# rqhuang88/DV-Matcher

Hardware: AMD Instinct MI355X
Metric: point-cloud pairs/sec (N=2048, d=128) (higher is better)
Workload: dtype f32; 1 GPU; BASELINE configs[1]: synthetic random pairs N=M=2048 d=128, correspondence+deform forward, both directions; deformer_weights=reference ckpt/dvmatcher_scape_r (fixture), fps_start=0, parallelism=pairs sharded over 1 GPU(s), no collective

## Files before the change

dv-matcher_amd/csrc/dvm_grid.hip:

```cpp
#include <stdlib.h>

#include <type_traits>

#include "dvm_common.h"
#include "dvm_mlp_f16.h"

namespace dvm {

constexpr int GRID_T = 256;

template <class IndexT>
struct GridViewT {
    const float4 *pts;
    const IndexT *ids;
    const IndexT *start;
    float ox, oy, oz, h, scale2;
    int G;
};
typedef GridViewT<int32_t> GridView;
typedef GridViewT<uint16_t> GridViewLds;


static int grid_dim_for(int P) {
    int g = 2;
    while (g < 16 && (double)(g + 1) * (g + 1) * (g + 1) * 1.2 <= (double)P * 1.15) ++g;
    return g < 4 ? 4 : g;
}

struct GridBuildSets {
    const float *xyz[4];
    int Nsrc[4];
    GridBuf gb[4];
};
template <bool SETS>
__device__ __forceinline__ void grid_build_body(const float *__restrict__ xyz, int Nsrc, const int32_t *__restrict__ sel, const GridBuf &gb);
__global__ __launch_bounds__(GRID_T) void grid_build_sets_kernel(const GridBuildSets sets) {
    const int q = blockIdx.y;
    grid_build_body<true>(sets.xyz[q], sets.Nsrc[q], nullptr, sets.gb[q]);
}
__global__ __launch_bounds__(GRID_T) void grid_build_kernel(const float *__restrict__ xyz, int Nsrc,
                                                            const int32_t *__restrict__ sel, GridBuf gb) {
    grid_build_body<false>(xyz, Nsrc, sel, gb);
}
template <bool SETS>
__device__ __forceinline__ void grid_build_body(const float *__restrict__ xyz, int Nsrc, const int32_t *__restrict__ sel, const GridBuf &gb) {
    extern __shared__ int lds[];
    __shared__ float red[6][GRID_T / 64];
    __shared__ float par[8];
    __shared__ int wsum[GRID_T / 64];
    const int b = blockIdx.x, tid = threadIdx.x, lane = tid & 63, wave = tid >> 6;
    const int P = gb.P, G = gb.G, G3 = G * G * G;
    const float *p = xyz + (size_t)b * Nsrc * 3;
    const int32_t *sl = sel ? sel + (size_t)b * P : nullptr;
    constexpr int GC = 8;
    const bool cached = P <= GC * GRID_T;
    float px[GC], py[GC], pz[GC];
    if (cached) {
        int vs[GC];
#pragma unroll
        for (int q = 0; q < GC; ++q) {
            const int j = tid + q * GRID_T, jc = j < P ? j : P - 1;
            vs[q] = sl ? sl[jc] : jc;
        }
#pragma unroll
        for (int q = 0; q < GC; ++q) px[q] = p[3 * vs[q]], py[q] = p[3 * vs[q] + 1], pz[q] = p[3 * vs[q] + 2];
    }
    auto each_point = [&](auto &&f) __attribute__((always_inline)) {
        if (cached) {
#pragma unroll
            for (int q = 0; q < GC; ++q) {
                const int j = tid + q * GRID_T;
                if (j < P) f(j, px[q], py[q], pz[q]);
            }
        } else {
            for (int j = tid; j < P; j += GRID_T) {
                const int v = sl ? sl[j] : j;
                f(j, p[3 * v], p[3 * v + 1], p[3 * v + 2]);
            }
        }
    };
    float mn[3] = {INFINITY, INFINITY, INFINITY}, mx[3] = {-INFINITY, -INFINITY, -INFINITY};
    each_point([&](int, float x, float y, float z) {
        mn[0] = fminf(mn[0], x), mn[1] = fminf(mn[1], y), mn[2] = fminf(mn[2], z);
        mx[0] = fmaxf(mx[0], x), mx[1] = fmaxf(mx[1], y), mx[2] = fmaxf(mx[2], z);
    });
    for (int a = 0; a < 3; ++a) {
        for (int o = 32; o > 0; o >>= 1) {
            mn[a] = fminf(mn[a], __shfl_xor(mn[a], o, 64));
            mx[a] = fmaxf(mx[a], __shfl_xor(mx[a], o, 64));
        }
        if (lane == 0) {
            red[a][wave] = mn[a];
            red[3 + a][wave] = mx[a];
        }
    }
    __syncthreads();
    if (tid == 0) {
        float lo[3], hi[3];
        for (int a = 0; a < 3; ++a) {
            lo[a] = fminf(fminf(red[a][0], red[a][1]), fminf(red[a][2], red[a][3]));
            hi[a] = fmaxf(fmaxf(red[3 + a][0], red[3 + a][1]), fmaxf(red[3 + a][2], red[3 + a][3]));
        }
        float ext = fmaxf(fmaxf(hi[0] - lo[0], hi[1] - lo[1]), hi[2] - lo[2]);
        float h = ext > 0.f ? (ext / (float)G) * 1.000001f : 1.f;
        float m = 0.f;
        for (int a = 0; a < 3; ++a) m = fmaxf(m, fmaxf(fabsf(lo[a]), fabsf(hi[a])));
        par[0] = lo[0], par[1] = lo[1], par[2] = lo[2], par[3] = h, par[4] = 3.f * m * m + 1e-30f;
        for (int q = 0; q < 5; ++q) gb.params[(size_t)b * 8 + q] = par[q];
    }
    for (int c = tid; c <= G3; c += GRID_T) lds[c] = 0;
    __syncthreads();
    const float ox = par[0], oy = par[1], oz = par[2], inv = 1.0f / par[3];
    auto cell_of = [&](float x, float y, float z) {
        int cx = (int)((x - ox) * inv), cy = (int)((y - oy) * inv), cz = (int)((z - oz) * inv);
        cx = cx < 0 ? 0 : (cx > G - 1 ? G - 1 : cx);
        cy = cy < 0 ? 0 : (cy > G - 1 ? G - 1 : cy);
        cz = cz < 0 ? 0 : (cz > G - 1 ? G - 1 : cz);
        return (cz * G + cy) * G + cx;
    };
    each_point([&](int, float x, float y, float z) { atomicAdd(&lds[cell_of(x, y, z)], 1); });
    __syncthreads();
    const int chunk = (G3 + GRID_T - 1) / GRID_T;
    int local = 0;
    for (int c = tid * chunk; c < (tid + 1) * chunk && c < G3; ++c) local += lds[c];
    int inc = local;
    for (int o = 1; o < 64; o <<= 1) {
        int t = __shfl_up(inc, o, 64);
        if (lane >= o) inc += t;
    }
    if (lane == 63) wsum[wave] = inc;
    __syncthreads();
    int base = inc - local;
    for (int w2 = 0; w2 < wave; ++w2) base += wsum[w2];
    __syncthreads();
    int *cursor = lds + G3 + 1;
    int run = base;
    for (int c = tid * chunk; c < (tid + 1) * chunk && c < G3; ++c) {
        int cnt = lds[c];
        lds[c] = run;
        cursor[c] = run;
        run += cnt;
    }
    if (tid == 0) lds[G3] = P;
    __syncthreads();
    int32_t *st = gb.start + (size_t)b * (G3 + 1);
    for (int c = tid; c <= G3; c += GRID_T) st[c] = lds[c];
    float4 *op = gb.pts + (size_t)b * P;
    int32_t *oi = gb.ids + (size_t)b * P;
    each_point([&](int j, float x, float y, float z) {
        const int pos = atomicAdd(&cursor[cell_of(x, y, z)], 1);
        op[pos] = make_float4(x, y, z, sumsq3(x, y, z));
        oi[pos] = j;
    });
}

__device__ __forceinline__ GridView grid_view(const GridBuf &gb, int b) {
    GridView g;
    const int G3 = gb.G * gb.G * gb.G;
    g.pts = gb.pts + (size_t)b * gb.P;
    g.ids = gb.ids + (size_t)b * gb.P;
    g.start = gb.start + (size_t)b * (G3 + 1);
    const float *pr = gb.params + (size_t)b * 8;
    g.ox = pr[0], g.oy = pr[1], g.oz = pr[2], g.h = pr[3], g.scale2 = pr[4];
    g.G = gb.G;
    return g;
}

struct MetricMMQueryRow {
    typedef float key_t;
    float qx, qy, qz, nq;
    __device__ __forceinline__ void set(float x, float y, float z) { qx = x, qy = y, qz = z, nq = sumsq3(x, y, z); }
    __device__ __forceinline__ float operator()(const float4 &c) const {
        return sqrt_rn(d2_mm3(qx, qy, qz, nq, c.x, c.y, c.z, c.w));
    }
    __device__ __forceinline__ static float to_d2(float k) { return k * k; }
};
struct MetricMMCandRow {
    typedef float key_t;
    float qx, qy, qz, nq;
    __device__ __forceinline__ void set(float x, float y, float z) { qx = x, qy = y, qz = z, nq = sumsq3(x, y, z); }
    __device__ __forceinline__ float operator()(const float4 &c) const {
        return sqrt_rn(d2_mm3(c.x, c.y, c.z, c.w, qx, qy, qz, nq));
    }
    __device__ __forceinline__ static float to_d2(float k) { return k * k; }
};
struct MetricF64 {
    typedef double key_t;
    float qx, qy, qz;
    __device__ __forceinline__ void set(float x, float y, float z) { qx = x, qy = y, qz = z; }
    __device__ __forceinline__ double operator()(const float4 &c) const {
        double dx = (double)qx - (double)c.x, dy = (double)qy - (double)c.y, dz = (double)qz - (double)c.z;
        double s = 0.0;
        s = s + dx * dx;
        s = s + dy * dy;
        s = s + dz * dz;
        return s;
    }
    __device__ __forceinline__ static float to_d2(double k) { return (float)k; }
};
struct MetricF64Rounded {
    typedef float key_t;
    MetricF64 m;
    __device__ __forceinline__ void set(float x, float y, float z) { m.set(x, y, z); }
    __device__ __forceinline__ float operator()(const float4 &c) const { return (float)m(c); }
    __device__ __forceinline__ static float to_d2(float k) { return k; }
};
struct MetricDiff {
    typedef float key_t;
    float qx, qy, qz;
    __device__ __forceinline__ void set(float x, float y, float z) { qx = x, qy = y, qz = z; }
    __device__ __forceinline__ float operator()(const float4 &c) const { return d2_diff3(qx, qy, qz, c.x, c.y, c.z); }
    __device__ __forceinline__ static float to_d2(float k) { return k; }
};

template <class View, class Metric, class List>
__device__ __forceinline__ void grid_row(const View &g, const Metric &met, List &kb, int s0, int s1) {
    for (int s = s0; s < s1; ++s) kb.insert_lex(met(g.pts[s]), (int)g.ids[s]);
}

struct ChamferMin {
    float key;
    __device__ __forceinline__ float worst() const { return key; }
};
template <class Metric>
__device__ __forceinline__ void grid_row(const GridView &g, const Metric &met, ChamferMin &kb, int s0, int s1) {
    for (; s0 < s1; s0 += 4) {
        float4 pc[4];
#pragma unroll
        for (int u = 0; u < 4; ++u) pc[u] = g.pts[s0 + u < s1 ? s0 + u : s1 - 1];
#pragma unroll
        for (int u = 0; u < 4; ++u) kb.key = fminf(kb.key, s0 + u < s1 ? met(pc[u]) : INFINITY);
    }
}
struct ChamferMinPos {
    float key;
    int pos;
    __device__ __forceinline__ float worst() const { return key; }
};
template <class Metric>
__device__ __forceinline__ void grid_row(const GridView &g, const Metric &met, ChamferMinPos &kb, int s0, int s1) {
    for (int s = s0; s < s1; ++s) {
        const float v = met(g.pts[s]);
        if (v < kb.key) {
            kb.key = v, kb.pos = s;
        } else if (v == kb.key && (kb.pos < 0 || g.ids[s] < g.ids[kb.pos])) {
            kb.pos = s;
        }
    }
}

template <int K, class Metric, class List, class View>
__device__ __forceinline__ bool grid_search(const View &g, float qx, float qy, float qz, Metric &met, List &kb,
                                            int R0 = 1 , int Rmax = 1 << 30) {
    const int G = g.G;
    const float inv = 1.0f / g.h;
    int cx = (int)((qx - g.ox) * inv), cy = (int)((qy - g.oy) * inv), cz = (int)((qz - g.oz) * inv);
    cx = cx < 0 ? 0 : (cx > G - 1 ? G - 1 : cx);
    cy = cy < 0 ? 0 : (cy > G - 1 ? G - 1 : cy);
    cz = cz < 0 ? 0 : (cz > G - 1 ? G - 1 : cz);
    const float q2 = sumsq3(qx, qy, qz);
    const float margin = 64.f * 1.1920929e-7f * (g.scale2 + q2) + 1e-30f;
    int Rprev = R0 > 1 ? R0 - 1 : -1;
    for (int R = R0; R <= G && R <= Rmax; ++R) {
        const int x0 = cx - R < 0 ? 0 : cx - R, x1 = cx + R > G - 1 ? G - 1 : cx + R;
        const int y0 = cy - R < 0 ? 0 : cy - R, y1 = cy + R > G - 1 ? G - 1 : cy + R;
        const int z0 = cz - R < 0 ? 0 : cz - R, z1 = cz + R > G - 1 ? G - 1 : cz + R;
        for (int z = z0; z <= z1; ++z) {
            const float zlo = g.oz + (float)z * g.h;
            const float dz = fmaxf(0.f, fmaxf(zlo - qz, qz - (zlo + g.h)));
            for (int y = y0; y <= y1; ++y) {
                const float ylo = g.oy + (float)y * g.h;
                const float dy = fmaxf(0.f, fmaxf(ylo - qy, qy - (ylo + g.h)));
                if (Metric::to_d2(kb.worst()) < (dy * dy + dz * dz) * 0.9999f - margin) continue;
                const int rowbase = (z * G + y) * G;
                const bool inner_zy = (abs(z - cz) <= Rprev) && (abs(y - cy) <= Rprev);
                int sa0, sa1, sb0 = 0, sb1 = 0;
                if (inner_zy) {
                    const int ix0 = cx - Rprev < 0 ? 0 : cx - Rprev;
                    const int ix1 = cx + Rprev > G - 1 ? G - 1 : cx + Rprev;
                    sa0 = g.start[rowbase + x0];
                    sa1 = g.start[rowbase + ix0];
                    sb0 = g.start[rowbase + ix1 + 1];
                    sb1 = g.start[rowbase + x1 + 1];
                } else {
                    sa0 = g.start[rowbase + x0];
                    sa1 = g.start[rowbase + x1 + 1];
                }
                grid_row(g, met, kb, sa0, sa1);
                grid_row(g, met, kb, sb0, sb1);
            }
        }
        const float ext = (float)G * g.h;
        const float ex = fmaxf(0.f, fmaxf(g.ox - qx, qx - (g.ox + ext)));
        const float ey = fmaxf(0.f, fmaxf(g.oy - qy, qy - (g.oy + ext)));
        const float ez = fmaxf(0.f, fmaxf(g.oz - qz, qz - (g.oz + ext)));
        const float exx = ex * ex, eyy = ey * ey, ezz = ez * ez;
        float bound2 = INFINITY;
        auto face_x = [&](float f) { f = fmaxf(f, 0.f); bound2 = fminf(bound2, f * f + eyy + ezz); };
        auto face_y = [&](float f) { f = fmaxf(f, 0.f); bound2 = fminf(bound2, f * f + exx + ezz); };
        auto face_z = [&](float f) { f = fmaxf(f, 0.f); bound2 = fminf(bound2, f * f + exx + eyy); };
        if (cx - R >= 1) face_x(qx - (g.ox + (float)(cx - R) * g.h));
        if (cx + R < G - 1) face_x((g.ox + (float)(cx + R + 1) * g.h) - qx);
        if (cy - R >= 1) face_y(qy - (g.oy + (float)(cy - R) * g.h));
        if (cy + R < G - 1) face_y((g.oy + (float)(cy + R + 1) * g.h) - qy);
        if (cz - R >= 1) face_z(qz - (g.oz + (float)(cz - R) * g.h));
        if (cz + R < G - 1) face_z((g.oz + (float)(cz + R + 1) * g.h) - qz);
        if (bound2 == INFINITY) return true;
        const float kth = Metric::to_d2(kb.worst());
        if (kth < bound2 * 0.9999f - margin) return true;
        Rprev = R;
    }
    return Rmax >= G;
}

static __host__ __device__ __forceinline__ size_t grid_lds_bytes(int P, int G) {
    return ((size_t)P * (sizeof(float4) + sizeof(uint16_t)) + ((size_t)G * G * G + 1) * sizeof(uint16_t) + 15) / 16 * 16;
}
static size_t grid_lds_bytes(const GridBuf &gb) { return gb.P < 65536 ? grid_lds_bytes(gb.P, gb.G) : ~(size_t)0; }
__device__ __forceinline__ GridViewLds grid_stage_lds(const GridView &g, int P, char *lds, int threads) {
    const int G3 = g.G * g.G * g.G;
    float4 *lp = (float4 *)lds;
    uint16_t *li = (uint16_t *)(lds + (size_t)P * sizeof(float4));
    uint16_t *ls = li + P;
    for (int i = threadIdx.x; i < P; i += threads) lp[i] = g.pts[i], li[i] = (uint16_t)g.ids[i];
    for (int i = threadIdx.x; i <= G3; i += threads) ls[i] = (uint16_t)g.start[i];
    GridViewLds v;
    v.pts = lp, v.ids = li, v.start = ls;
    v.ox = g.ox, v.oy = g.oy, v.oz = g.oz, v.h = g.h, v.scale2 = g.scale2, v.G = g.G;
    return v;
}

template <int K, int THREADS = 128, bool LDS_GRID = false>
__global__ __launch_bounds__(THREADS) void grid_knn_self_kernel(GridBuf gb, int k, int32_t *__restrict__ idx) {
    extern __shared__ __attribute__((aligned(16))) char kn_lds[];
    const int b = blockIdx.y;
    const int t = blockIdx.x * blockDim.x + threadIdx.x;
    const int P = gb.P;
    const GridView gg = grid_view(gb, b);
    typename std::conditional<LDS_GRID, GridViewLds, GridView>::type g;
    if constexpr (LDS_GRID) {
        g = grid_stage_lds(gg, P, kn_lds, THREADS);
        __syncthreads();
    } else {
        g = gg;
    }
    if (t >= P) return;
    const float4 qp = g.pts[t];
    MetricMMQueryRow met;
    met.set(qp.x, qp.y, qp.z);
    KBestPacked<K> kb;
    kb.init(INFINITY);
    grid_search<K, MetricMMQueryRow>(g, qp.x, qp.y, qp.z, met, kb);
    int32_t *o = idx + ((size_t)b * P + g.ids[t]) * k;
    for (int q = 0; q < K; ++q)
        if (q < k) o[q] = (unsigned)kb.idx_at(q) < (unsigned)P ? kb.idx_at(q) : 0;
}

template <int THREADS = 128, bool LDS_GRID = false>
__global__ __launch_bounds__(THREADS) void grid_ring_kernel(GridBuf gb, int32_t *__restrict__ ring) {
    extern __shared__ __attribute__((aligned(16))) char rg_lds[];
    const int b = blockIdx.y;
    const int t = blockIdx.x * blockDim.x + threadIdx.x;
    const int P = gb.P;
    const GridView gg = grid_view(gb, b);
    typename std::conditional<LDS_GRID, GridViewLds, GridView>::type g;
    if constexpr (LDS_GRID) {
        g = grid_stage_lds(gg, P, rg_lds, THREADS);
        __syncthreads();
    } else {
        g = gg;
    }
    if (t >= P) return;
    const float4 qp = g.pts[t];
    const int a = g.ids[t];
    int32_t *o = ring + ((size_t)b * P + a) * 9;
    MetricF64Rounded mr;
    mr.set(qp.x, qp.y, qp.z);
    KBestPacked<10, 8> ks;
    ks.init(INFINITY);
    grid_search<9, MetricF64Rounded>(g, qp.x, qp.y, qp.z, mr, ks);
    bool ambiguous = false;
#pragma unroll
    for (int q = 0; q < 9; ++q) ambiguous = ambiguous || (ks.key_at(q) == ks.key_at(q + 1) && ks.key_at(q) < INFINITY);
    if (!ambiguous) {
        for (int q = 0; q < 9; ++q) o[q] = (unsigned)ks.idx_at(q) < (unsigned)P ? ks.idx_at(q) : a;
        return;
    }
    MetricF64 met;
    met.set(qp.x, qp.y, qp.z);
    KBest<9, double> kb;
    kb.init((double)INFINITY);
    grid_search<9, MetricF64>(g, qp.x, qp.y, qp.z, met, kb);
    for (int q = 0; q < 9; ++q) o[q] = (unsigned)kb.idx[q] < (unsigned)P ? kb.idx[q] : a;
}

template <int THREADS = 128, int LDS_GRID = 0>
__global__ __launch_bounds__(THREADS) void grid_infl_kernel(const float *__restrict__ xyz, int N, GridBuf gnodes, GridBuf gverts,
                                                            int32_t *__restrict__ infl, float *__restrict__ dists,
                                                            double *__restrict__ nnd) {
    extern __shared__ __attribute__((aligned(16))) char in_lds[];
    const int b = blockIdx.y;
    const int t = blockIdx.x * blockDim.x + threadIdx.x;
    const GridView gv0 = grid_view(gverts, b), gn0 = grid_view(gnodes, b);
    typename std::conditional<(LDS_GRID & 2) != 0, GridViewLds, GridView>::type gv;
    typename std::conditional<(LDS_GRID & 1) != 0, GridViewLds, GridView>::type gn;
    size_t used = 0;
    if constexpr ((LDS_GRID & 2) != 0) {
        gv = grid_stage_lds(gv0, gverts.P, in_lds, THREADS);
        used = grid_lds_bytes(gverts.P, gverts.G);
    } else {
        gv = gv0;
    }
    if constexpr ((LDS_GRID & 1) != 0) {
        gn = grid_stage_lds(gn0, gnodes.P, in_lds + used, THREADS);
    } else {
        gn = gn0;
    }
    if (LDS_GRID) __syncthreads();
    if (t >= N) return;
    const float4 qp = gv.pts[t];
    const int i = gv.ids[t];
    {
        MetricMMCandRow met;
        met.set(qp.x, qp.y, qp.z);
        KBestPacked<3> kb;
        kb.init(INFINITY);
        grid_search<3, MetricMMCandRow>(gn, qp.x, qp.y, qp.z, met, kb);
        const size_t row = (size_t)b * N + i;
        for (int q = 0; q < 3; ++q) {
            infl[row * 3 + q] = (unsigned)kb.idx_at(q) < (unsigned)gnodes.P ? kb.idx_at(q) : 0;
            dists[row * 3 + q] = kb.key_at(q);
        }
    }
    {
        MetricF64 met;
        met.set(qp.x, qp.y, qp.z);
        KBest<2, double> kb;
        kb.init((double)INFINITY);
        grid_search<2, MetricF64>(gv, qp.x, qp.y, qp.z, met, kb);
        nnd[(size_t)b * N + i] = sqrt(kb.key[1]);
    }
    (void)xyz;
}

struct ChGridGroup {
    GridBuf gq;
    GridBuf gb;
    float *dout;
    int32_t *iout;
};
struct ChGridArgs {
    ChGridGroup g[8];
    int scan_min;
    unsigned long long *stats;
};
typedef float f32x16_g __attribute__((ext_vector_type(16)));
typedef _Float16 f16x8_g __attribute__((ext_vector_type(8)));
typedef unsigned u32x4_g __attribute__((ext_vector_type(4)));

template <bool WANT_IDX>
__device__ __forceinline__ void chamfer_exact_scan(const GridView &g, const MetricDiff &met, int s_begin, int s_end, float &best, int &bs) {
    for (int s0 = s_begin; s0 < s_end; s0 += 4) {
        float4 pc[4];
#pragma unroll
        for (int u = 0; u < 4; ++u) pc[u] = g.pts[s0 + u < s_end ? s0 + u : s_end - 1];
#pragma unroll
        for (int u = 0; u < 4; ++u) {
            const int sidx = s0 + u;
            const float d = sidx < s_end ? met(pc[u]) : INFINITY;
            if (!WANT_IDX) {
                best = fminf(best, d);
            } else if (d < best) {
                best = d, bs = sidx;
            } else if (d == best && d < INFINITY && g.ids[sidx] < g.ids[bs]) {
                bs = sidx;
            }
        }
    }
}

__device__ __forceinline__ float fmin2i(float a, float b) {
    float r;
    asm("v_min_f32 %0, %1, %2" : "=v"(r) : "v"(a), "v"(b));
    return r;
}
__device__ __forceinline__ float acc_min16(const f32x16_g &acc, float inf) {
    const float last = __builtin_canonicalizef(acc[15]);
    float r0, r1, r2;
    asm("v_min3_f32 %0, %3, %4, %5\n\t"
        "v_min3_f32 %1, %6, %7, %8\n\t"
        "v_min3_f32 %2, %9, %10, %11\n\t"
        "v_min3_f32 %0, %0, %1, %2\n\t"
        "v_min3_f32 %1, %12, %13, %14\n\t"
        "v_min3_f32 %2, %15, %16, %17\n\t"
        "v_min3_f32 %1, %1, %2, %18\n\t"
        "v_min3_f32 %0, %0, %1, %19"
        : "=&v"(r0), "=&v"(r1), "=&v"(r2)
        : "v"(acc[0]), "v"(acc[1]), "v"(acc[2]), "v"(acc[3]), "v"(acc[4]), "v"(acc[5]), "v"(acc[6]), "v"(acc[7]), "v"(acc[8]),
          "v"(acc[9]), "v"(acc[10]), "v"(acc[11]), "v"(acc[12]), "v"(acc[13]), "v"(acc[14]), "v"(last), "v"(inf));
    return r0;
}
__device__ __forceinline__ float fmed3i(float a, float b, float c) {
    float r;
    asm("v_med3_f32 %0, %1, %2, %3" : "=v"(r) : "v"(a), "v"(b), "v"(c));
    return r;
}

template <bool WANT_IDX>
__device__ __forceinline__ void chamfer_scan_wave(const ChGridGroup &G, const GridView &g, int b, int Na, bool done, const float4 qp, int i,
                                                  const MetricDiff &met, float margin, unsigned long long *stats, int grp) {
    const int P = G.gb.P;
    const int lane = threadIdx.x & 63, j32 = lane & 31, hh = lane >> 5;
    if (stats) {
        if (lane == 0) atomicAdd(stats + grp * 8 + 5, 1ull);
        if (!done) atomicAdd(stats + grp * 8 + 6, 1ull);
    }
    float tb[2] = {INFINITY, INFINITY}, ts[2] = {INFINITY, INFINITY}, th[2] = {INFINITY, INFINITY};
    int tt[2] = {0, 0}, tu[2] = {0, 0};
    const float finf = INFINITY;
    auto keep = [&](int tl, float m, int s0) {
        const bool lt1 = m < tb[tl], lt2 = m < ts[tl];
        int tun = lt2 ? s0 : tu[tl];
        asm volatile("" : "+v"(tun));
        tu[tl] = lt1 ? tt[tl] : tun;
        tt[tl] = lt1 ? s0 : tt[tl];
        th[tl] = fmed3i(ts[tl], th[tl], m);
        ts[tl] = fmed3i(tb[tl], ts[tl], m);
        tb[tl] = fmin2i(tb[tl], m);
    };
    constexpr int TB = 2;
    auto fetch = [&](float4 (&buf)[TB], int s00) {
#pragma unroll
        for (int u = 0; u < TB; ++u) {
            const int pi = s00 + j32, last = P - 1 - 32 * u;
            buf[u] = g.pts[(pi < last ? pi : last) + 32 * u];
        }
    };
    auto sweep = [&](auto &&unit) {
        float4 pa[TB], pb[TB];
        fetch(pa, 0);
        for (int s00 = 0; s00 < P; s00 += 64 * TB) {
            fetch(pb, s00 + 32 * TB);
#pragma unroll
            for (int u = 0; u < TB; ++u) {
                if (s00 + 32 * u >= P) break;
                unit(pa[u], s00 + 32 * u);
            }
            fetch(pa, s00 + 64 * TB);
#pragma unroll
            for (int u = 0; u < TB; ++u) {
                if (s00 + 32 * (TB + u) >= P) break;
                unit(pb[u], s00 + 32 * (TB + u));
            }
        }
    };
    float q2m = sumsq3(qp.x, qp.y, qp.z);
#pragma unroll
    for (int o = 32; o > 0; o >>= 1) q2m = fmaxf(q2m, __shfl_xor(q2m, o, 64));
    const int r2bits = __builtin_amdgcn_readfirstlane(__float_as_int(fmaxf(g.scale2, q2m)));
    const bool f16 = r2bits < 0x7f800000;
    const int ks = (25 - ((r2bits >> 23) - 127)) >> 1;
    const float sc2 = f16 ? __int_as_float((2 * ks + 127) << 23) : 1.f;
    if (f16) {
        const float sq = __int_as_float((ks + 127) << 23), sx = -2.f * sq, sn = __int_as_float((2 * ks - 12 + 127) << 23);
        f16x8_g bq[2];
#pragma unroll
        for (int tl = 0; tl < 2; ++tl) {
            const int src = j32 + 32 * tl;
            const float x = __shfl(qp.x, src, 64), y = __shfl(qp.y, src, 64), z = __shfl(qp.z, src, 64);
            unsigned h01, m01, h23, m23;
            split2x2(sq * x, sq * y, h01, m01);
            split2x2(sq * z, 4096.f, h23, m23);
            bq[tl] = __builtin_bit_cast(f16x8_g, u32x4_g{hh ? 0u : h01, hh ? 0u : h23, hh ? m01 : h01, hh ? m23 : h23});
        }
        sweep([&](const float4 &pc, int s0) {
            unsigned h01, m01, h23, m23;
            split2x2(sx * pc.x, sx * pc.y, h01, m01);
            split2x2(sx * pc.z, sn * pc.w, h23, m23);
            const f16x8_g a = __builtin_bit_cast(f16x8_g, u32x4_g{hh ? 0u : h01, hh ? 0u : h23, hh ? h01 : m01, hh ? h23 : m23});
            const f32x16_g zero = {0.f, 0.f, 0.f, 0.f, 0.f, 0.f, 0.f, 0.f, 0.f, 0.f, 0.f, 0.f, 0.f, 0.f, 0.f, 0.f};
            const f32x16_g acc0 = __builtin_amdgcn_mfma_f32_32x32x16_f16(a, bq[0], zero, 0, 0, 0);
            const f32x16_g acc1 = __builtin_amdgcn_mfma_f32_32x32x16_f16(a, bq[1], zero, 0, 0, 0);
            keep(0, acc_min16(acc0, finf), s0);
            keep(1, acc_min16(acc1, finf), s0);
        });
    } else {
        float bq[2][2];
#pragma unroll
        for (int tl = 0; tl < 2; ++tl) {
            const int src = j32 + 32 * tl;
            const float x = __shfl(qp.x, src, 64), y = __shfl(qp.y, src, 64), z = __shfl(qp.z, src, 64);
            bq[tl][0] = hh ? -2.f * y : -2.f * x;
            bq[tl][1] = hh ? 1.f : -2.f * z;
        }
        sweep([&](const float4 &pc, int s0) {
            const float a0 = hh ? pc.y : pc.x, a1 = hh ? pc.w : pc.z;
#pragma unroll
            for (int tl = 0; tl < 2; ++tl) {
                f32x16_g acc = {0.f, 0.f, 0.f, 0.f, 0.f, 0.f, 0.f, 0.f, 0.f, 0.f, 0.f, 0.f, 0.f, 0.f, 0.f, 0.f};
                acc = __builtin_amdgcn_mfma_f32_32x32x2f32(a0, bq[tl][0], acc, 0, 0, 0);
                acc = __builtin_amdgcn_mfma_f32_32x32x2f32(a1, bq[tl][1], acc, 0, 0, 0);
                keep(tl, acc_min16(acc, finf), s0);
            }
        });
    }
    const float b1 = hh ? tb[1] : tb[0], s1 = hh ? ts[1] : ts[0], h1 = hh ? th[1] : th[0];
    const int t1 = hh ? tt[1] : tt[0], u1 = hh ? tu[1] : tu[0];
    const float b2 = __shfl_xor(hh ? tb[0] : tb[1], 32, 64), s2 = __shfl_xor(hh ? ts[0] : ts[1], 32, 64), h2 = __shfl_xor(hh ? th[0] : th[1], 32, 64);
    const int t2 = __shfl_xor(hh ? tt[0] : tt[1], 32, 64), u2 = __shfl_xor(hh ? tu[0] : tu[1], 32, 64);
    const float sbest = fminf(b1, b2);
    const int stile = b2 < b1 ? t2 : t1;
    const float c1 = t1 != stile ? b1 : INFINITY, c2 = u1 != stile ? s1 : INFINITY, c3 = t2 != stile ? b2 : INFINITY, c4 = u2 != stile ? s2 : INFINITY;
    const float ssec = fminf(fminf(c1, c2), fminf(c3, c4));
    const int stile2 = ssec == c1 ? t1 : (ssec == c2 ? u1 : (ssec == c3 ? t2 : u2));
    const float o1 = t1 != stile2 ? c1 : INFINITY, o2 = u1 != stile2 ? c2 : INFINITY, o3 = t2 != stile2 ? c3 : INFINITY, o4 = u2 != stile2 ? c4 : INFINITY;
    const float sother = fminf(fminf(h1, h2), fminf(fminf(o1, o2), fminf(o3, o4)));
    float best = INFINITY;
    int bs = 0;
    bool cert = false;
    if (!done) {
        chamfer_exact_scan<WANT_IDX>(g, met, stile, stile + 32 < P ? stile + 32 : P, best, bs);
        if (ssec < INFINITY) chamfer_exact_scan<WANT_IDX>(g, met, stile2, stile2 + 32 < P ? stile2 + 32 : P, best, bs);
        cert = sother - sbest > 2.f * (f16 ? margin * sc2 + 4.f : margin);
    }
    if (__ballot(!done && !cert) != 0) {
        if (!done && !cert) {
            if (stats) atomicAdd(stats + grp * 8 + 7, 1ull);
            best = INFINITY, bs = 0;
            chamfer_exact_scan<WANT_IDX>(g, met, 0, P, best, bs);
        }
    }
    if (!done) {
        G.dout[(size_t)b * Na + i] = best;
        if (WANT_IDX && G.iout) G.iout[(size_t)b * Na + i] = g.ids[bs];
    }
}

template <int THREADS, bool LDS_TARGET, bool WANT_IDX>
__global__ __launch_bounds__(THREADS) void grid_chamfer_kernel(const ChGridArgs args) {
    extern __shared__ __attribute__((aligned(16))) char ch_lds[];
    const ChGridGroup &G = args.g[blockIdx.z];
    const int b = blockIdx.y;
    const int t = blockIdx.x * blockDim.x + threadIdx.x;
    const int Na = G.gq.P;
    const bool inrange = t < Na;
    GridView g = grid_view(G.gb, b);
    if (LDS_TARGET) {
        const int P = G.gb.P, G3 = G.gb.G * G.gb.G * G.gb.G;
        float4 *lp = (float4 *)ch_lds;
        int32_t *ls = (int32_t *)(ch_lds + (size_t)P * sizeof(float4));
        for (int i = threadIdx.x; i < P; i += THREADS) lp[i] = g.pts[i];
        for (int i = threadIdx.x; i <= G3; i += THREADS) ls[i] = g.start[i];
        __syncthreads();
        g.pts = lp;
        g.start = ls;
    }
    GridView q = grid_view(G.gq, b);
    const int tq = inrange ? t : Na - 1;
    const float4 qp = q.pts[tq];
    const int i = q.ids[tq];
    MetricDiff met;
    met.set(qp.x, qp.y, qp.z);
    const float q2 = sumsq3(qp.x, qp.y, qp.z);
    const float margin = 64.f * 1.1920929e-7f * (g.scale2 + q2) + 1e-30f;
    bool done = !inrange;
    float fbest = INFINITY;
    int fpos = -1;
    {
        const int Gd = g.G;
        const float inv = 1.0f / g.h;
        int cx = (int)((qp.x - g.ox) * inv), cy = (int)((qp.y - g.oy) * inv), cz = (int)((qp.z - g.oz) * inv);
        cx = cx < 0 ? 0 : (cx > Gd - 1 ? Gd - 1 : cx);
        cy = cy < 0 ? 0 : (cy > Gd - 1 ? Gd - 1 : cy);
        cz = cz < 0 ? 0 : (cz > Gd - 1 ? Gd - 1 : cz);
        const int x0 = cx - 1 < 0 ? 0 : cx - 1, x1 = cx + 1 > Gd - 1 ? Gd - 1 : cx + 1;
        int rs[9], re[9];
#pragma unroll
        for (int r = 0; r < 9; ++r) {
            const int z = cz + r / 3 - 1, y = cy + r % 3 - 1;
            const bool in = z >= 0 && z < Gd && y >= 0 && y < Gd;
            const int rowbase = ((in ? z : cz) * Gd + (in ? y : cy)) * Gd;
            rs[r] = g.start[rowbase + x0];
            const int rend = g.start[rowbase + x1 + 1];
            re[r] = in ? rend : rs[r];
        }
        float best = INFINITY;
        int bs = -1;
        bool tie = false;
        const float dlo[2] = {fmaxf(0.f, qp.y - (g.oy + (float)cy * g.h)), fmaxf(0.f, qp.z - (g.oz + (float)cz * g.h))};
        const float dhi[2] = {fmaxf(0.f, (g.oy + (float)(cy + 1) * g.h) - qp.y), fmaxf(0.f, (g.oz + (float)(cz + 1) * g.h) - qp.z)};
        constexpr int order[9] = {4, 1, 3, 5, 7, 0, 2, 6, 8};
        float rowb[9];
#pragma unroll
        for (int r = 0; r < 9; ++r) {
            const float dyr = r % 3 == 1 ? 0.f : (r % 3 == 0 ? dlo[0] : dhi[0]), dzr = r / 3 == 1 ? 0.f : (r / 3 == 0 ? dlo[1] : dhi[1]);
            rowb[r] = (dyr * dyr + dzr * dzr) * 0.9999f - margin;
        }
#pragma unroll
        for (int ri = 0; ri < 9; ++ri) {
            const int r = order[ri];
            if (best < rowb[r]) continue;
            const int rend = re[r];
            for (int s0 = rs[r]; s0 < rend; s0 += 4) {
                float4 pc[4];
#pragma unroll
                for (int u = 0; u < 4; ++u) pc[u] = g.pts[s0 + u < rend ? s0 + u : rend - 1];
#pragma unroll
                for (int u = 0; u < 4; ++u) {
                    const int s = s0 + u;
                    float dm = met(pc[u]);
                    asm volatile("" : "+v"(dm));
                    const bool inb = s < rend;
                    const float d = inb ? dm : INFINITY;
                    if (WANT_IDX) {
                        const bool lt = d < best, eq = d == best && inb && d < INFINITY;
                        tie = lt ? false : (tie || eq);
                        bs = lt ? s : bs;
                        best = lt ? d : best;
                    } else {
                        best = fminf(best, d);
                    }
                }
            }
        }
        if (WANT_IDX && tie && bs >= 0) {
            int bid = g.ids[bs];
#pragma unroll 1
            for (int r = 0; r < 9; ++r) {
                if (best < rowb[r]) continue;
                for (int s = rs[r]; s < re[r]; ++s) {
                    if (met(g.pts[s]) == best) {
                        const int id = g.ids[s];
                        if (id < bid) bid = id, bs = s;
                    }
                }
            }
        }
        const float ext = (float)Gd * g.h;
        const float ex = fmaxf(0.f, fmaxf(g.ox - qp.x, qp.x - (g.ox + ext)));
        const float ey = fmaxf(0.f, fmaxf(g.oy - qp.y, qp.y - (g.oy + ext)));
        const float ez = fmaxf(0.f, fmaxf(g.oz - qp.z, qp.z - (g.oz + ext)));
        const float exx = ex * ex, eyy = ey * ey, ezz = ez * ez;
        float bound2 = INFINITY;
        auto face = [&](float f, float o2) { f = fmaxf(f, 0.f); bound2 = fminf(bound2, f * f + o2); };
        if (cx - 1 >= 1) face(qp.x - (g.ox + (float)(cx - 1) * g.h), eyy + ezz);
        if (cx + 1 < Gd - 1) face((g.ox + (float)(cx + 2) * g.h) - qp.x, eyy + ezz);
        if (cy - 1 >= 1) face(qp.y - (g.oy + (float)(cy - 1) * g.h), exx + ezz);
        if (cy + 1 < Gd - 1) face((g.oy + (float)(cy + 2) * g.h) - qp.y, exx + ezz);
        if (cz - 1 >= 1) face(qp.z - (g.oz + (float)(cz - 1) * g.h), exx + eyy);
        if (cz + 1 < Gd - 1) face((g.oz + (float)(cz + 2) * g.h) - qp.z, exx + eyy);
        if (args.stats && inrange) {
            int ncand = 0;
#pragma unroll
            for (int r = 0; r < 9; ++r) ncand += re[r] - rs[r];
            atomicAdd(args.stats + blockIdx.z * 8 + 0, 1ull);
            atomicAdd(args.stats + blockIdx.z * 8 + 1, (unsigned long long)ncand);
        }
        const bool found = WANT_IDX ? bs >= 0 : best < INFINITY;
        if (found) fbest = best, fpos = bs;
        if (!done && found && (bound2 == INFINITY || best < bound2 * 0.9999f - margin)) {
            G.dout[(size_t)b * Na + i] = best;
            if (WANT_IDX && G.iout) G.iout[(size_t)b * Na + i] = g.ids[bs];
            done = true;
            if (args.stats) atomicAdd(args.stats + blockIdx.z * 8 + 2, 1ull);
        }
    }
    const int nfall = __popcll(__ballot(!done));
    if (nfall == 0) return;
    bool scan = nfall >= args.scan_min;
    if (!scan) {
        if (!done) {
            if (args.stats) atomicAdd(args.stats + blockIdx.z * 8 + 3, 1ull);
            typename std::conditional<WANT_IDX, ChamferMinPos, ChamferMin>::type kb;
            kb.key = fbest;
            if constexpr (WANT_IDX) kb.pos = fpos;
            if (grid_search<1, MetricDiff>(g, qp.x, qp.y, qp.z, met, kb, 2, 3)) {
                if (args.stats) atomicAdd(args.stats + blockIdx.z * 8 + 4, 1ull);
                G.dout[(size_t)b * Na + i] = kb.key;
                if constexpr (WANT_IDX)
                    if (G.iout) G.iout[(size_t)b * Na + i] = kb.pos >= 0 ? g.ids[kb.pos] : 0;
                done = true;
            }
        }
        scan = __ballot(!done) != 0;
        if (!scan) return;
    }
    chamfer_scan_wave<WANT_IDX>(G, g, b, Na, done, qp, i, met, margin, args.stats, blockIdx.z);
}

GridBuf grid_carve(Arena &ar, int B, int P) {
    GridBuf gb;
    gb.P = P;
    gb.G = grid_dim_for(P);
    const int G3 = gb.G * gb.G * gb.G;
    gb.pts = ar.take<float4>((size_t)B * P);
    gb.ids = ar.take<int32_t>((size_t)B * P);
    gb.start = ar.take<int32_t>((size_t)B * (G3 + 1));
    gb.params = ar.take<float>((size_t)B * 8);
    return gb;
}
size_t grid_bytes(int B, int P) {
    Arena ar(nullptr, 0);
    grid_carve(ar, B, P);
    return ar.off;
}

void launch_grid_build_sets(const float *const *xyz, const int *Nsrc, const GridBuf *gb, int nsets, int B, hipStream_t s) {
    GridBuildSets sets;
    size_t lds = 0;
    for (int q = 0; q < 4; ++q) {
        const int r = q < nsets ? q : 0;
        sets.xyz[q] = xyz[r], sets.Nsrc[q] = Nsrc[r], sets.gb[q] = gb[r];
        const int G3 = gb[r].G * gb[r].G * gb[r].G;
        const size_t nb = (size_t)(2 * G3 + 1) * sizeof(int);
        lds = nb > lds ? nb : lds;
    }
    hipLaunchKernelGGL(grid_build_sets_kernel, dim3(B, nsets), dim3(GRID_T), lds, s, sets);
}
void launch_grid_build(const float *xyz, int B, int Nsrc, const int32_t *sel, const GridBuf &gb, hipStream_t s) {
    const int G3 = gb.G * gb.G * gb.G;
    size_t lds = (size_t)(2 * G3 + 1) * sizeof(int);
    hipLaunchKernelGGL(grid_build_kernel, dim3(B), dim3(GRID_T), lds, s, xyz, Nsrc, sel, gb);
}

template <int K>
static void launch_knn_self_k(const GridBuf &gb, int B, int k, int32_t *idx, hipStream_t s) {
    const size_t lds = grid_lds_bytes(gb);
    if (lds <= 64 * 1024) {
        ensure_dyn_lds((const void *)grid_knn_self_kernel<K, 512, true>, (int)lds);
        hipLaunchKernelGGL((grid_knn_self_kernel<K, 512, true>), dim3((gb.P + 511) / 512, B), dim3(512), lds, s, gb, k, idx);
    } else {
        hipLaunchKernelGGL((grid_knn_self_kernel<K, 128, false>), dim3((gb.P + 127) / 128, B), dim3(128), 0, s, gb, k, idx);
    }
}

void launch_grid_knn_self(const GridBuf &gb, int B, int k, int32_t *idx, hipStream_t s) {
    prof_begin(s, DVM_PROF_KNN_XYZ);
    if (k <= 3)
        launch_knn_self_k<3>(gb, B, k, idx, s);
    else if (k <= 10)
        launch_knn_self_k<10>(gb, B, k, idx, s);
    else
        launch_knn_self_k<16>(gb, B, k, idx, s);
    prof_end(s, DVM_PROF_KNN_XYZ);
}

void launch_grid_ring(const GridBuf &gnodes, int B, int32_t *ring, hipStream_t s) {
    const size_t lds = grid_lds_bytes(gnodes);
    if (lds <= 64 * 1024) {
        ensure_dyn_lds((const void *)grid_ring_kernel<512, true>, (int)lds);
        hipLaunchKernelGGL((grid_ring_kernel<512, true>), dim3((gnodes.P + 511) / 512, B), dim3(512), lds, s, gnodes, ring);
    } else {
        hipLaunchKernelGGL((grid_ring_kernel<128, false>), dim3((gnodes.P + 127) / 128, B), dim3(128), 0, s, gnodes, ring);
    }
}

void launch_grid_infl(const float *xyz, int B, int N, const GridBuf &gnodes, const GridBuf &gverts, int32_t *infl, float *dists,
                      double *nnd, hipStream_t s) {
    const size_t lds = grid_lds_bytes(gnodes);
    if (lds <= 64 * 1024) {
        ensure_dyn_lds((const void *)grid_infl_kernel<512, 1>, (int)lds);
        hipLaunchKernelGGL((grid_infl_kernel<512, 1>), dim3((N + 511) / 512, B), dim3(512), lds, s, xyz, N, gnodes, gverts, infl, dists, nnd);
    } else {
        hipLaunchKernelGGL((grid_infl_kernel<128, 0>), dim3((N + 127) / 128, B), dim3(128), 0, s, xyz, N, gnodes, gverts, infl, dists, nnd);
    }
}

void launch_grid_chamfer(const GridBuf *gq, const GridBuf *gb, float *const *dout, int32_t *const *iout, int ngroups, int B,
                         hipStream_t s) {
    ChGridArgs args;
    int maxN = 1;
    for (int q = 0; q < 8; ++q) {
        int r = q < ngroups ? q : 0;
        args.g[q] = ChGridGroup{gq[r], gb[r], dout[r], iout ? iout[r] : nullptr};
        if (q < ngroups && gq[r].P > maxN) maxN = gq[r].P;
    }
    bool want_idx = false;
    for (int q = 0; q < ngroups; ++q) want_idx = want_idx || args.g[q].iout != nullptr;
    args.scan_min = 24;
    args.stats = nullptr;
    if ((options().debug & DVM_DEBUG_CHAMFER_STATS) && hipMalloc(&args.stats, 64 * sizeof(unsigned long long)) == hipSuccess)
        (void)hipMemsetAsync(args.stats, 0, 64 * sizeof(unsigned long long), s);
    size_t lds_bytes = 0;
    for (int q = 0; q < ngroups; ++q) {
        const size_t nb = (size_t)gb[q].P * sizeof(float4) + ((size_t)gb[q].G * gb[q].G * gb[q].G + 1) * sizeof(int32_t);
        lds_bytes = nb > lds_bytes ? nb : lds_bytes;
    }
    lds_bytes = (lds_bytes + 15) / 16 * 16;
    prof_begin(s, DVM_PROF_CHAMFER);
    const dim3 grid_lds((maxN + 511) / 512, B, ngroups), grid_glb((maxN + 127) / 128, B, ngroups);
    if (lds_bytes <= 64 * 1024 && want_idx) {
        ensure_dyn_lds((const void *)grid_chamfer_kernel<512, true, true>, (int)lds_bytes);
        hipLaunchKernelGGL((grid_chamfer_kernel<512, true, true>), grid_lds, dim3(512), lds_bytes, s, args);
    } else if (lds_bytes <= 64 * 1024) {
        ensure_dyn_lds((const void *)grid_chamfer_kernel<512, true, false>, (int)lds_bytes);
        hipLaunchKernelGGL((grid_chamfer_kernel<512, true, false>), grid_lds, dim3(512), lds_bytes, s, args);
    } else if (want_idx) {
        hipLaunchKernelGGL((grid_chamfer_kernel<128, false, true>), grid_glb, dim3(128), 0, s, args);
    } else {
        hipLaunchKernelGGL((grid_chamfer_kernel<128, false, false>), grid_glb, dim3(128), 0, s, args);
    }
    prof_end(s, DVM_PROF_CHAMFER);
    if (args.stats) {
        unsigned long long h[64];
        (void)hipStreamSynchronize(s);
        (void)hipMemcpy(h, args.stats, sizeof(h), hipMemcpyDeviceToHost);
        for (int q = 0; q < ngroups; ++q)
            fprintf(stderr, "chamfer group %d: %llu queries, %.1f radius-1 candidates each, %.1f%% certified there, %.1f%% walked (%.1f%% certified by the walk), "
                            "%llu waves scanned for %llu lanes, %llu exact fallbacks\n", q, h[q * 8], (double)h[q * 8 + 1] / (double)(h[q * 8] ? h[q * 8] : 1),
                    100.0 * h[q * 8 + 2] / (h[q * 8] ? h[q * 8] : 1), 100.0 * h[q * 8 + 3] / (h[q * 8] ? h[q * 8] : 1),
                    100.0 * h[q * 8 + 4] / (h[q * 8] ? h[q * 8] : 1), h[q * 8 + 5], h[q * 8 + 6], h[q * 8 + 7]);
        (void)hipFree(args.stats);
    }
}

}
```

Before: 58770 pairs/s.

## Compact unresolved chamfer queries before MFMA scan and gate scan by work units

Before the wave-wide MFMA brute-force scan, the lanes whose nearest neighbour is still unresolved are packed to the front of the wavefront with ds_permute. When 32 or fewer remain, a single-half variant issues one MFMA per tile instead of two. The scan-versus-grid-fallback decision now also limits halves times tiles to a scan_units budget of 128, so large targets fall back to the grid search. This adds permute overhead and another template instantiation, and the grid fallback can be slower on waves that would previously have scanned.

Result: no change. 58510 pairs/s (-0.4%).

```diff
diff --git a/dv-matcher_amd/csrc/dvm_grid.hip b/dv-matcher_amd/csrc/dvm_grid.hip
--- a/dv-matcher_amd/csrc/dvm_grid.hip
+++ b/dv-matcher_amd/csrc/dvm_grid.hip
@@ -451,9 +451,10 @@
 };
 struct ChGridArgs {
     ChGridGroup g[8];
-    int scan_min;
+    int scan_min, scan_units;
     unsigned long long *stats;
 };
+__device__ __forceinline__ float chamfer_margin(float scale2, float q2) { return 64.f * 1.1920929e-7f * (scale2 + q2) + 1e-30f; }
 typedef float f32x16_g __attribute__((ext_vector_type(16)));
 typedef _Float16 f16x8_g __attribute__((ext_vector_type(8)));
 typedef unsigned u32x4_g __attribute__((ext_vector_type(4)));
@@ -506,11 +507,12 @@
     return r;
 }
 
-template <bool WANT_IDX>
-__device__ __forceinline__ void chamfer_scan_wave(const ChGridGroup &G, const GridView &g, int b, int Na, bool done, const float4 qp, int i,
+template <bool WANT_IDX, int NH>
+__device__ __forceinline__ void chamfer_scan_wave(const ChGridGroup &G, const GridView &g, int b, int Na, int nopen, const float4 qp, int i,
                                                   const MetricDiff &met, float margin, unsigned long long *stats, int grp) {
     const int P = G.gb.P;
     const int lane = threadIdx.x & 63, j32 = lane & 31, hh = lane >> 5;
+    const bool done = lane >= nopen;
     if (stats) {
         if (lane == 0) atomicAdd(stats + grp * 8 + 5, 1ull);
         if (!done) atomicAdd(stats + grp * 8 + 6, 1ull);
@@ -565,7 +567,7 @@
         const float sq = __int_as_float((ks + 127) << 23), sx = -2.f * sq, sn = __int_as_float((2 * ks - 12 + 127) << 23);
         f16x8_g bq[2];
 #pragma unroll
-        for (int tl = 0; tl < 2; ++tl) {
+        for (int tl = 0; tl < NH; ++tl) {
             const int src = j32 + 32 * tl;
             const float x = __shfl(qp.x, src, 64), y = __shfl(qp.y, src, 64), z = __shfl(qp.z, src, 64);
             unsigned h01, m01, h23, m23;
@@ -580,14 +582,18 @@
             const f16x8_g a = __builtin_bit_cast(f16x8_g, u32x4_g{hh ? 0u : h01, hh ? 0u : h23, hh ? h01 : m01, hh ? h23 : m23});
             const f32x16_g zero = {0.f, 0.f, 0.f, 0.f, 0.f, 0.f, 0.f, 0.f, 0.f, 0.f, 0.f, 0.f, 0.f, 0.f, 0.f, 0.f};
             const f32x16_g acc0 = __builtin_amdgcn_mfma_f32_32x32x16_f16(a, bq[0], zero, 0, 0, 0);
-            const f32x16_g acc1 = __builtin_amdgcn_mfma_f32_32x32x16_f16(a, bq[1], zero, 0, 0, 0);
-            keep(0, acc_min16(acc0, finf), s0);
-            keep(1, acc_min16(acc1, finf), s0);
+            if constexpr (NH == 2) {
+                const f32x16_g acc1 = __builtin_amdgcn_mfma_f32_32x32x16_f16(a, bq[1], zero, 0, 0, 0);
+                keep(0, acc_min16(acc0, finf), s0);
+                keep(1, acc_min16(acc1, finf), s0);
+            } else {
+                keep(0, acc_min16(acc0, finf), s0);
+            }
         });
     } else {
         float bq[2][2];
 #pragma unroll
-        for (int tl = 0; tl < 2; ++tl) {
+        for (int tl = 0; tl < NH; ++tl) {
             const int src = j32 + 32 * tl;
             const float x = __shfl(qp.x, src, 64), y = __shfl(qp.y, src, 64), z = __shfl(qp.z, src, 64);
             bq[tl][0] = hh ? -2.f * y : -2.f * x;
@@ -596,7 +602,7 @@
         sweep([&](const float4 &pc, int s0) {
             const float a0 = hh ? pc.y : pc.x, a1 = hh ? pc.w : pc.z;
 #pragma unroll
-            for (int tl = 0; tl < 2; ++tl) {
+            for (int tl = 0; tl < NH; ++tl) {
                 f32x16_g acc = {0.f, 0.f, 0.f, 0.f, 0.f, 0.f, 0.f, 0.f, 0.f, 0.f, 0.f, 0.f, 0.f, 0.f, 0.f, 0.f};
                 acc = __builtin_amdgcn_mfma_f32_32x32x2f32(a0, bq[tl][0], acc, 0, 0, 0);
                 acc = __builtin_amdgcn_mfma_f32_32x32x2f32(a1, bq[tl][1], acc, 0, 0, 0);
@@ -604,10 +610,12 @@
             }
         });
     }
-    const float b1 = hh ? tb[1] : tb[0], s1 = hh ? ts[1] : ts[0], h1 = hh ? th[1] : th[0];
-    const int t1 = hh ? tt[1] : tt[0], u1 = hh ? tu[1] : tu[0];
-    const float b2 = __shfl_xor(hh ? tb[0] : tb[1], 32, 64), s2 = __shfl_xor(hh ? ts[0] : ts[1], 32, 64), h2 = __shfl_xor(hh ? th[0] : th[1], 32, 64);
-    const int t2 = __shfl_xor(hh ? tt[0] : tt[1], 32, 64), u2 = __shfl_xor(hh ? tu[0] : tu[1], 32, 64);
+    const bool own1 = NH == 2 && hh;
+    const float b1 = own1 ? tb[1] : tb[0], s1 = own1 ? ts[1] : ts[0], h1 = own1 ? th[1] : th[0];
+    const int t1 = own1 ? tt[1] : tt[0], u1 = own1 ? tu[1] : tu[0];
+    const bool oth1 = NH == 2 && !hh;
+    const float b2 = __shfl_xor(oth1 ? tb[1] : tb[0], 32, 64), s2 = __shfl_xor(oth1 ? ts[1] : ts[0], 32, 64), h2 = __shfl_xor(oth1 ? th[1] : th[0], 32, 64);
+    const int t2 = __shfl_xor(oth1 ? tt[1] : tt[0], 32, 64), u2 = __shfl_xor(oth1 ? tu[1] : tu[0], 32, 64);
     const float sbest = fminf(b1, b2);
     const int stile = b2 < b1 ? t2 : t1;
     const float c1 = t1 != stile ? b1 : INFINITY, c2 = u1 != stile ? s1 : INFINITY, c3 = t2 != stile ? b2 : INFINITY, c4 = u2 != stile ? s2 : INFINITY;
@@ -634,6 +642,30 @@
         G.dout[(size_t)b * Na + i] = best;
         if (WANT_IDX && G.iout) G.iout[(size_t)b * Na + i] = g.ids[bs];
     }
+}
+
+template <bool WANT_IDX>
+__device__ __forceinline__ void chamfer_scan_open(const ChGridGroup &G, const GridView &g, int b, int Na, bool done, float4 qp, int i,
+                                                  unsigned long long *stats, int grp) {
+    const unsigned long long open = __ballot(!done);
+    const int nopen = __popcll(open);
+    const int lane = threadIdx.x & 63;
+    const int below = (int)__builtin_amdgcn_mbcnt_hi((unsigned)(open >> 32), __builtin_amdgcn_mbcnt_lo((unsigned)open, 0u));
+    const int dst = (done ? nopen + (lane - below) : below) << 2;
+    const int mx = __builtin_amdgcn_ds_permute(dst, __float_as_int(qp.x)), my = __builtin_amdgcn_ds_permute(dst, __float_as_int(qp.y));
+    const int mz = __builtin_amdgcn_ds_permute(dst, __float_as_int(qp.z)), mi = __builtin_amdgcn_ds_permute(dst, i);
+    const bool mine = lane < nopen;
+    qp.x = __int_as_float(mine ? mx : __builtin_amdgcn_readfirstlane(mx));
+    qp.y = __int_as_float(mine ? my : __builtin_amdgcn_readfirstlane(my));
+    qp.z = __int_as_float(mine ? mz : __builtin_amdgcn_readfirstlane(mz));
+    i = mine ? mi : __builtin_amdgcn_readfirstlane(mi);
+    MetricDiff met;
+    met.set(qp.x, qp.y, qp.z);
+    const float margin = chamfer_margin(g.scale2, sumsq3(qp.x, qp.y, qp.z));
+    if (nopen <= 32)
+        chamfer_scan_wave<WANT_IDX, 1>(G, g, b, Na, nopen, qp, i, met, margin, stats, grp);
+    else
+        chamfer_scan_wave<WANT_IDX, 2>(G, g, b, Na, nopen, qp, i, met, margin, stats, grp);
 }
 
 template <int THREADS, bool LDS_TARGET, bool WANT_IDX>
@@ -661,8 +693,7 @@
     const int i = q.ids[tq];
     MetricDiff met;
     met.set(qp.x, qp.y, qp.z);
-    const float q2 = sumsq3(qp.x, qp.y, qp.z);
-    const float margin = 64.f * 1.1920929e-7f * (g.scale2 + q2) + 1e-30f;
+    const float margin = chamfer_margin(g.scale2, sumsq3(qp.x, qp.y, qp.z));
     bool done = !inrange;
     float fbest = INFINITY;
     int fpos = -1;
@@ -767,7 +798,8 @@
     }
     const int nfall = __popcll(__ballot(!done));
     if (nfall == 0) return;
-    bool scan = nfall >= args.scan_min;
+    const int halves = (nfall + 31) >> 5, tiles = (G.gb.P + 31) >> 5;
+    bool scan = nfall >= args.scan_min && halves * tiles <= args.scan_units;
     if (!scan) {
         if (!done) {
             if (args.stats) atomicAdd(args.stats + blockIdx.z * 8 + 3, 1ull);
@@ -785,7 +817,7 @@
         scan = __ballot(!done) != 0;
         if (!scan) return;
     }
-    chamfer_scan_wave<WANT_IDX>(G, g, b, Na, done, qp, i, met, margin, args.stats, blockIdx.z);
+    chamfer_scan_open<WANT_IDX>(G, g, b, Na, done, qp, i, args.stats, blockIdx.z);
 }
 
 GridBuf grid_carve(Arena &ar, int B, int P) {
@@ -878,6 +910,7 @@
     bool want_idx = false;
     for (int q = 0; q < ngroups; ++q) want_idx = want_idx || args.g[q].iout != nullptr;
     args.scan_min = 24;
+    args.scan_units = 128;
     args.stats = nullptr;
     if ((options().debug & DVM_DEBUG_CHAMFER_STATS) && hipMalloc(&args.stats, 64 * sizeof(unsigned long long)) == hipSuccess)
         (void)hipMemsetAsync(args.stats, 0, 64 * sizeof(unsigned long long), s);
```
